# PRBonn/SHINE_mapping

Hardware: NVIDIA H100
Metric: sdf_train_points_per_sec_fwd_bwd (higher is better)
Workload: dtype f32

## Files before the change

### shine_mapping_b200/csrc/shine_b200.cu

```cuda

#include <cuda_runtime.h>
#include <math.h>
#include <stdint.h>

#include <type_traits>

#include "shine_b200.h"

#ifndef SHINE_GATHER_GROUP
#define SHINE_GATHER_GROUP 2
#endif
#ifndef SHINE_TRAIN_MINB
#define SHINE_TRAIN_MINB 2
#endif
#ifndef SHINE_TRAIN_DECGRAD_MINB
#define SHINE_TRAIN_DECGRAD_MINB 1
#endif
#ifndef SHINE_INFER_MINB
#define SHINE_INFER_MINB 3
#endif

#include "shine_device.cuh"

namespace {
// ... 205 lines not shown
                    acc.x = fmaf(w, v.x, acc.x); acc.y = fmaf(w, v.y, acc.y); acc.z = fmaf(w, v.z, acc.z); acc.w = fmaf(w, v.w, acc.w);
                } else {
                    red_add_f4(lv.feature_grads + (int64_t)ids[c] * F + 4 * part, w * d.x, w * d.y, w * d.z, w * d.w);
                }
            }
        }
    }
    if (MODE == 0) {
#pragma unroll
        for (int o = 1; o < LP; o <<= 1) {
            g3[0] += __shfl_xor_sync(kFull, g3[0], o); g3[1] += __shfl_xor_sync(kFull, g3[1], o); g3[2] += __shfl_xor_sync(kFull, g3[2], o);
        }
        if (valid && part == 0) { out[3 * p] = g3[0]; out[3 * p + 1] = g3[1]; out[3 * p + 2] = g3[2]; }
    } else if (MODE == 1) {
        if (valid) *reinterpret_cast<float4*>(out + p * F + 4 * part) = acc;
    }
}

__device__ __forceinline__ void to_afrag(const float (&v)[4], int odd, float (&a)[4]) {
    const float s0 = odd ? v[0] : v[2], s1 = odd ? v[1] : v[3];
    const float r0 = __shfl_xor_sync(kFull, s0, 1), r1 = __shfl_xor_sync(kFull, s1, 1);
    if (!odd) { a[0] = v[0]; a[2] = v[1]; a[1] = r0; a[3] = r1; }
    else      { a[0] = r0;   a[2] = r1;   a[1] = v[2]; a[3] = v[3]; }
}
__device__ __forceinline__ void from_cfrag(const float (&c)[4], int odd, float (&v)[4]) {
    const float s0 = odd ? c[0] : c[2], s1 = odd ? c[1] : c[3];
    const float r0 = __shfl_xor_sync(kFull, s0, 1), r1 = __shfl_xor_sync(kFull, s1, 1);
    if (!odd) { v[0] = c[0]; v[1] = c[1]; v[2] = r0; v[3] = r1; }
    else      { v[0] = r0;   v[1] = r1;   v[2] = c[2]; v[3] = c[3]; }
}

#define SHINE_ACC_DECL float dW2[2][4][4], dW1[2][4], db2p[4][2], db1p[4][2], dw3p[4][2]

__device__ __forceinline__ float reduce_scatter_g8(const float (&v)[8], int lane) {
    float a[4], b[2];
    const bool b4 = (lane & 16) != 0, b3 = (lane & 8) != 0, b2 = (lane & 4) != 0;
#pragma unroll
    for (int i = 0; i < 4; ++i) a[i] = (b4 ? v[4 + i] : v[i]) + __shfl_xor_sync(kFull, b4 ? v[i] : v[4 + i], 16);
#pragma unroll
    for (int i = 0; i < 2; ++i) b[i] = (b3 ? a[2 + i] : a[i]) + __shfl_xor_sync(kFull, b3 ? a[i] : a[2 + i], 8);
    return (b2 ? b[1] : b[0]) + __shfl_xor_sync(kFull, b2 ? b[0] : b[1], 4);
}

__device__ __forceinline__ int frag_chunk(int lane) { return lane ^ ((lane >> 2) & 6); }
template <int NTF>
__device__ __forceinline__ void load_afrag(const float* blk, int c, AFrag<NTF>& a) {
    const float4 v = *reinterpret_cast<const float4*>(blk + 4 * c);
    a.set_packed(v.x, v.y, v.z, v.w);
}
__device__ __forceinline__ void load_bfrag(const float* blk, int c, uint2& bh, uint2& bl) {
    const float2 v = *reinterpret_cast<const float2*>(blk + 2 * c);
    split_fast2(v.x, v.y, bh.x, bh.y, bl.x, bl.y);
}
__device__ __forceinline__ void stage_afrags(float* blk, const int (&sq)[2], const float (&c)[4][4]) {
#pragma unroll
    for (int mt = 0; mt < 2; ++mt)
#pragma unroll
        for (int q = 0; q < 2; ++q)
            *reinterpret_cast<float4*>(blk + 128 * mt + 4 * sq[q]) = make_float4(c[2 * mt][q], c[2 * mt + 1][q], c[2 * mt][2 + q], c[2 * mt + 1][2 + q]);
}
__device__ __forceinline__ int xfrag_word(int ks, int c) { return 64 * ks + 2 * (c ^ (8 * ks)); }
__device__ __forceinline__ void load_xfrag(const float* sx, int ks, int c, uint2& bh, uint2& bl) {
    const float2 v = *reinterpret_cast<const float2*>(sx + xfrag_word(ks, c));
    split_fast2(v.x, v.y, bh.x, bh.y, bl.x, bl.y);
}


constexpr int kGatherGroup = SHINE_GATHER_GROUP;

using shine_internal::StepParams;

struct SmemPlan {
    static constexpr int W1 = 0;
    static constexpr int W1T = W1 + 2 * kH * kF;
    static constexpr int W2 = W1T + 2 * kF * kWS;
    static constexpr int W3W2T = W2 + 2 * kH * kWS;
    static constexpr int B1 = W3W2T + 2 * kH * kWS;
    static constexpr int B2 = B1 + kH;
    static constexpr int W3 = B2 + kH;
    static constexpr int B3 = W3 + kH;
    static constexpr int GSCALE = B3 + 1;
    static constexpr int kDecGradFloats = kH * kF + kH + kH * kH + kH + kH + 1;
    static constexpr int ZSUM = B3 + 4;
    static constexpr int kZsumFloats = 8 * 5 * kTile;
    static constexpr int STAGE = ZSUM + kZsumFloats;
    static constexpr int SB2 = 0;
    static constexpr int SU = SB2;
    static constexpr int SA1 = SB2 + kTile * kH;
    static constexpr int SX = SA1 + kTile * kH;
    static constexpr int SA2 = SX + kTile * kF;
    static constexpr int SDP = SA2;
    static constexpr int kStagePerWarp = SA2 + kTile * kH;
    static constexpr int kStageGrouped = SDP + 2 * kTile;
    __host__ __device__ static constexpr int stage_per_warp(bool grouped) { return grouped ? kStageGrouped : kStagePerWarp; }
    static constexpr int kGroupPerLevel = 4 * kTile;
    static constexpr int kW2Part = kH * kH;
};

constexpr int kMaxGroupedRuns = 6;

__device__ __forceinline__ void red_add_f2(float* p, float a, float b) {
    asm volatile("red.global.add.v2.f32 [%0], {%1,%2};" ::"l"(p), "f"(a), "f"(b) : "memory");
}
__device__ __forceinline__ int group_slot(int p) { return 4 * (p & 3) + (p >> 2); }

template <int LMAX>
__device__ __forceinline__ void grouped_scatter(const StepParams& P, int L, int tile, const float* __restrict__ pt,
                                                float* __restrict__ dtile, const float (&dxc)[4], int lane) {
    const int g = lane >> 2, t = lane & 3;
    *reinterpret_cast<float2*>(dtile + g * kF + 2 * t) = make_float2(dxc[0], dxc[1]);
    *reinterpret_cast<float2*>(dtile + (g + 8) * kF + 2 * t) = make_float2(dxc[2], dxc[3]);
    __syncwarp();
    uint2 bh[2], bl[2];
#pragma unroll
    for (int c = 0; c < 2; ++c)
        split_fast2(dtile[(8 * c + t) * kF + g], dtile[(8 * c + t + 4) * kF + g], bh[c].x, bh[c].y, bl[c].x, bl[c].y);
    const float sx = (g & 4) ? 1.f : -1.f, ox = (g & 4) ? 0.f : 1.f;
    const float sy = (g & 2) ? 1.f : -1.f, oy = (g & 2) ? 0.f : 1.f;
    const float sz = (g & 1) ? 1.f : -1.f, oz = (g & 1) ? 0.f : 1.f;
    const int id_off = 8 * (g & 1) + 4 + (g >> 1);
    const int own = group_slot(lane & 15);
#pragma unroll
    for (int i = 0; i < LMAX; ++i) {
        if (i >= L) break;
        const float* lt = pt + i * SmemPlan::kGroupPerLevel;
        const int v_own = __float_as_int(lt[48 + own]);
        const uint32_t same = __match_any_sync(kFull, v_own);
        const int lead = __ffs(same) - 1;
        const uint32_t bmask = __ballot_sync(kFull, v_own >= 0 && lead == lane);
        if (bmask == 0) continue;
        const int rid_own = v_own >= 0 ? __popc(bmask & ((1u << lead) - 1u)) : 255;
        const shine_level& lv = P.oct.lv[i];
        const int32_t* slot_words = reinterpret_cast<const int32_t*>(lv.hash_slots);
        float* gb = grad_base(lv, (uint32_t)tile, kF);
        const int nruns = __popc(bmask);
        if (nruns > kMaxGroupedRuns) {
            const int odd = t & 1, half = t >> 1, mp = group_slot(g + 8 * odd);
            const int v = __float_as_int(lt[48 + mp]);
            if (v >= 0) {
                const float tx = lt[mp], ty = lt[16 + mp], tz = lt[32 + mp];
                const float ux = __fsub_rn(1.0f, tx), uy = __fsub_rn(1.0f, ty), uz = __fsub_rn(1.0f, tz);
                const int4 e = ldg_i4(slot_words + 16 * (int64_t)v + 4), o = ldg_i4(slot_words + 16 * (int64_t)v + 12);
                const int ids[8] = {e.x, o.x, e.y, o.y, e.z, o.z, e.w, o.w};
                const float4 d = *reinterpret_cast<const float4*>(dtile + (g + 8 * odd) * kF + 4 * half);
                const float xy[4] = {__fmul_rn(ux, uy), __fmul_rn(ux, ty), __fmul_rn(tx, uy), __fmul_rn(tx, ty)};
                const f2_t zz = f2_pack(uz, tz), d01 = f2_pack(d.x, d.y), d23 = f2_pack(d.z, d.w);
#pragma unroll
                for (int c = 0; c < 8; c += 2) {
                    float w[2];
                    f2_unpack(f2_mul(f2_pack(xy[c >> 1], xy[c >> 1]), zz), w[0], w[1]);
#pragma unroll
                    for (int k = 0; k < 2; ++k) {
                        const f2_t wk = f2_pack(w[k], w[k]);
                        float g0, g1, g2, g3;
                        f2_unpack(f2_mul(wk, d01), g0, g1); f2_unpack(f2_mul(wk, d23), g2, g3);
                        red_add_f4(gb + (int64_t)ids[c + k] * kF + 4 * half, g0, g1, g2, g3);
                    }
                }
            }
            continue;
        }
        const float4 tx4 = *reinterpret_cast<const float4*>(lt + 4 * t);
        const float4 ty4 = *reinterpret_cast<const float4*>(lt + 16 + 4 * t);
        const float4 tz4 = *reinterpret_cast<const float4*>(lt + 32 + 4 * t);
        float w[4];
        {
            const f2_t s_x = f2_pack(sx, sx), o_x = f2_pack(ox, ox), s_y = f2_pack(sy, sy), o_y = f2_pack(oy, oy);
            const f2_t s_z = f2_pack(sz, sz), o_z = f2_pack(oz, oz);
            const f2_t X01 = f2_fma(f2_pack(tx4.x, tx4.y), s_x, o_x), X23 = f2_fma(f2_pack(tx4.z, tx4.w), s_x, o_x);
            const f2_t Y01 = f2_fma(f2_pack(ty4.x, ty4.y), s_y, o_y), Y23 = f2_fma(f2_pack(ty4.z, ty4.w), s_y, o_y);
            const f2_t Z01 = f2_fma(f2_pack(tz4.x, tz4.y), s_z, o_z), Z23 = f2_fma(f2_pack(tz4.z, tz4.w), s_z, o_z);
            f2_unpack(f2_mul(f2_mul(X01, Y01), Z01), w[0], w[1]);
            f2_unpack(f2_mul(f2_mul(X23, Y23), Z23), w[2], w[3]);
        }
        int rid[4];
#pragma unroll
        for (int q = 0; q < 4; ++q) rid[q] = __shfl_sync(kFull, rid_own, t + 4 * q);
        uint32_t rem = bmask;
        for (int r = 0; r < nruns; r += 2) {
            const int p1 = __ffs(rem) - 1; rem &= rem - 1;
// ... 60 lines not shown
    const int g = lane >> 2, t = lane & 3, odd = t & 1, half = t >> 1;
    constexpr int kWarps = 8;

    for (int i = tid; i < kH * kF; i += blockDim.x) {
        const int nrow = i / kF, k = i % kF;
        uint32_t hi, lo; split_tf32(P.dec.w1[i], hi, lo);
        smu[SmemPlan::W1 + i] = hi; smu[SmemPlan::W1 + kH * kF + i] = lo;
        smu[SmemPlan::W1T + k * kWS + nrow] = hi; smu[SmemPlan::W1T + kF * kWS + k * kWS + nrow] = lo;
    }
    for (int i = tid; i < kH * kH; i += blockDim.x) {
        const int nrow = i / kH, k = i % kH;
        const float w = P.dec.w2[i];
        uint32_t hi, lo; split_tf32(w, hi, lo);
        smu[SmemPlan::W2 + nrow * kWS + k] = hi; smu[SmemPlan::W2 + kH * kWS + nrow * kWS + k] = lo;
        split_tf32(__fmul_rn(P.dec.w3[nrow], w), hi, lo);
        smu[SmemPlan::W3W2T + k * kWS + nrow] = hi; smu[SmemPlan::W3W2T + kH * kWS + k * kWS + nrow] = lo;
    }
    if (tid < kH) {
        smem[SmemPlan::B1 + tid] = P.dec.b1 ? P.dec.b1[tid] : 0.f;
        smem[SmemPlan::B2 + tid] = P.dec.b2 ? P.dec.b2[tid] : 0.f;
        smem[SmemPlan::W3 + tid] = P.dec.w3[tid];
    }
    if (tid == 0) {
        smem[SmemPlan::B3] = P.dec.b3 ? P.dec.b3[0] : 0.f;
        smem[SmemPlan::GSCALE] = P.loss_scale * ((TRAIN && P.d_loss) ? __ldg(P.d_loss) : 1.0f);
    }
    constexpr int kPark = LMAX <= 4 ? 16 : 32;
    constexpr int kIdPark = 4 * LMAX;
    __syncthreads();
    SHINE_ACC_DECL;
#pragma unroll
    for (int a = 0; a < 2; ++a) {
#pragma unroll
        for (int b = 0; b < 4; ++b) { dW2[a][b][0] = dW2[a][b][1] = dW2[a][b][2] = dW2[a][b][3] = 0.f; }
        dW1[a][0] = dW1[a][1] = dW1[a][2] = dW1[a][3] = 0.f;
    }
#pragma unroll
    for (int j = 0; j < 4; ++j) { db2p[j][0] = db2p[j][1] = db1p[j][0] = db1p[j][1] = dw3p[j][0] = dw3p[j][1] = 0.f; }
    float dw3acc = 0.f, db2acc[4] = {0.f, 0.f, 0.f, 0.f}, db1acc[2][2] = {{0.f, 0.f}, {0.f, 0.f}};

    constexpr bool kSectorProbe = !TRAIN;
    const bool poly = P.oct.poly_interp != 0;
    const int L = P.oct.num_levels;

    float db3p = 0.f;
    float loss_acc = 0.f;

    constexpr int kStage = SmemPlan::stage_per_warp(GROUPED);
    float* stage = smem + SmemPlan::STAGE + warp * kStage;
    float* stX = stage + SmemPlan::SX;
    const int kp = g >> 2, fc = frag_chunk(lane);
    const int sq[2] = {frag_chunk(8 * t + (g & 3)), frag_chunk(8 * t + 4 + (g & 3))};
    float* gpt = smem + SmemPlan::STAGE + (DEC_GRAD ? 8 * kStage : 0) +
                 warp * (LMAX * SmemPlan::kGroupPerLevel + (DEC_GRAD ? 0 : kTile * kF));
    float* gdx = DEC_GRAD ? stX : gpt + LMAX * SmemPlan::kGroupPerLevel;
    float* w2p = smem + SmemPlan::STAGE + 8 * kStage + 8 * LMAX * SmemPlan::kGroupPerLevel + warp * SmemPlan::kW2Part;
    if (DEC_GRAD && GROUPED) {
#pragma unroll
        for (int f = 0; f < 8; ++f) *reinterpret_cast<float4*>(w2p + 128 * f + 4 * lane) = make_float4(0.f, 0.f, 0.f, 0.f);
    }

    const int warp_global = blockIdx.x * kWarps + warp;
    const int warp_stride = gridDim.x * kWarps;

    bool consecutive = true;
#pragma unroll
    for (int i = 1; i < LMAX; ++i)
        if (i < L && P.oct.lv[i].level != P.oct.lv[0].level - i) consecutive = false;

    float nx = 0.f, ny = 0.f, nz = 0.f, nlab = 0.f, nwgt = 1.f;
    bool nvalid = false;
    auto prefetch_inputs = [&](int tl) {
        const int64_t p = (int64_t)tl * kTile + g + 8 * odd;
        nvalid = tl < P.num_tiles && p < P.n;
        if (nvalid) {
            src.load(P, p, nx, ny, nz);
            if (P.label) nlab = __ldg(P.label + p);
            if (P.weighted) nwgt = fabsf(__ldg(P.weight + p));
        }
    };
    prefetch_inputs(warp_global);

    int phase = 0;
    bool advance = false, last_pass = false;
    float pred0 = 0.f, zsum = 0.f;
    auto loss_point = [&](float pv, float lb, float wg, float& li, float& dp) {
        if constexpr (LOSS == kLossBce) {
            const float zt = __fdividef(1.0f, 1.0f + __expf(-__fdividef(lb, P.sigma)));
            const float e = __expf(-fabsf(pv));
            li = fmaxf(pv, 0.f) - pv * zt + __logf(1.0f + e);
            dp = 0.f;
            if (TRAIN) {
                const float rs = __fdividef(1.0f, 1.0f + e);
                const float sg = pv >= 0.f ? rs : e * rs;
                dp = (sg - zt) * wg * smem[SmemPlan::GSCALE];
            }
        } else {
            float dli;
            diff_point<LOSS>(pv, lb, P.scale, li, dli);
            dp = TRAIN ? dli * wg * smem[SmemPlan::GSCALE] : 0.f;
        }
    };
    for (int seq = warp_global;; seq = advance ? seq + warp_stride : seq) {
        if (last_pass) break;
        const int tile = seq;
        if (phase == 1 && seq >= P.num_tiles) {
            if constexpr (DEC_GRAD) {
#pragma unroll
                for (int o = 16; o > 0; o >>= 1) zsum += __shfl_xor_sync(kFull, zsum, o);
                if (lane == 0) smem[SmemPlan::ZSUM + warp] = zsum;
                __syncthreads();
                if (warp != 0) break;
                float tot = 0.f;
#pragma unroll
                for (int w = 0; w < kWarps; ++w) tot += smem[SmemPlan::ZSUM + w];
                if (tot == 0.f) break;
                zsum = tot;
                phase = 2;
            } else {
                break;
            }
        }
        const bool virt = phase != 1;
        last_pass = phase == 2;
        advance = !virt;
        const int64_t base = (int64_t)tile * kTile;
        const int64_t myp = base + g + 8 * odd;
        const bool valid = virt ? false : nvalid;
        const float x = nx, y = ny, z = nz, lab = nlab, wgt = nwgt;
        if (!virt) prefetch_inputs(seq + warp_stride);

        float feat[4];
        float pk[kPark];
        float idp[kIdPark];
        uint32_t hitmask = 0;
        if constexpr (kSectorProbe) {
        {
            float acc[8] = {0.f, 0.f, 0.f, 0.f, 0.f, 0.f, 0.f, 0.f};
#pragma unroll
            for (int i = 0; i < kPark; ++i) pk[i] = 0.f;
            const unsigned long long key0 = valid ? morton_of(x, y, z, P.oct.lv[0].level) : 0ull;
#pragma unroll
            for (int g0 = 0; g0 < LMAX; g0 += kGatherGroup) {
                SlotSector sec[kGatherGroup];
#pragma unroll
                for (int j = 0; j < kGatherGroup; ++j) {
                    const int i = g0 + j;
                    if (i < L && valid) {
                        const shine_level& lv = P.oct.lv[i];
                        const unsigned long long kq = consecutive ? (key0 >> (3 * i)) : morton_of(x, y, z, lv.level);
                        sec[j] = ldg_sector(reinterpret_cast<const HashSlot*>(lv.hash_slots),
                                            hash_key(kq) & (lv.hash_capacity - 1), half);
                    }
                }
#pragma unroll
                for (int j = 0; j < kGatherGroup; ++j) {
                    const int i = g0 + j;
                    bool hit = false;
                    if (i < L && valid) {
                        const shine_level& lv = P.oct.lv[i];
                        const unsigned long long kq = consecutive ? (key0 >> (3 * i)) : morton_of(x, y, z, lv.level);
                        hit = resolve_sector(reinterpret_cast<const HashSlot*>(lv.hash_slots), lv.hash_capacity - 1, kq, half,
                                             sec[j]);
                    }
                    idp[4 * i] = __int_as_float(hit ? sec[j].ids[0] : -1); idp[4 * i + 1] = __int_as_float(hit ? sec[j].ids[1] : -1);
                    idp[4 * i + 2] = __int_as_float(hit ? sec[j].ids[2] : -1); idp[4 * i + 3] = __int_as_float(hit ? sec[j].ids[3] : -1);
                    if (hit) {
                        const shine_level& lv = P.oct.lv[i];
                        hitmask |= 1u << i;
                        float r0[8], r1[8], r2[8], r3[8];
                        ldg_row8(lv.features + (int64_t)sec[j].ids[0] * kF, r0);
                        ldg_row8(lv.features + (int64_t)sec[j].ids[1] * kF, r1);
                        ldg_row8(lv.features + (int64_t)sec[j].ids[2] * kF, r2);
                        ldg_row8(lv.features + (int64_t)sec[j].ids[3] * kF, r3);
                        Blend b; b.init(x, y, z, lv.level, poly);
                        pk[3 * i] = b.tx; pk[3 * i + 1] = b.ty; pk[3 * i + 2] = b.tz;
                        const float wz = half ? b.tz : b.uz;
                        const float w0 = __fmul_rn(__fmul_rn(b.ux, b.uy), wz), w1 = __fmul_rn(__fmul_rn(b.ux, b.ty), wz);
                        const float w2 = __fmul_rn(__fmul_rn(b.tx, b.uy), wz), w3 = __fmul_rn(__fmul_rn(b.tx, b.ty), wz);
                        blend4(acc, r0, r1, r2, r3, w0, w1, w2, w3);
                    }
                }
            }
#pragma unroll
            for (int q = 0; q < 4; ++q) {
                const float send = half ? acc[q] : acc[4 + q];
                const float recv = __shfl_xor_sync(kFull, send, 2);
                feat[q] = (half ? acc[4 + q] : acc[q]) + recv;
            }
        }
        } else {
        int slot[LMAX];
        {
            constexpr int LH = LMAX / 2;
            const unsigned long long key0 = valid ? morton_of(x, y, z, P.oct.lv[0].level) : 0ull;
            unsigned long long kq[LH];
            uint4 kf[LH];
            int mine[LH];
#pragma unroll
            for (int j = 0; j < LH; ++j) {
                const int i = 2 * j + half;
                mine[j] = -1;
                if (i < L && valid) {
                    const shine_level& lv = P.oct.lv[i];
                    const HashSlot* slots = reinterpret_cast<const HashSlot*>(lv.hash_slots);
                    kq[j] = consecutive ? (key0 >> (3 * i)) : morton_of(x, y, z, lv.level);
                    mine[j] = (int)(hash_key(kq[j]) & (lv.hash_capacity - 1));
// ... 91 lines not shown
        if (DEC_GRAD) {
#pragma unroll
            for (int q = 0; q < 4; ++q) stX[xfrag_word(kp, frag_chunk(16 * half + 4 * q + (g & 3))) + odd] = feat[q];
        }
        float h1[4][4];
        uint32_t m1 = 0;
        {
            uint2 bh[4], bl[4];
#pragma unroll
            for (int j = 0; j < 4; ++j) {
                const float bA = smem[SmemPlan::B1 + 8 * j + 2 * t], bB = smem[SmemPlan::B1 + 8 * j + 2 * t + 1];
                h1[j][0] = bA; h1[j][1] = bB; h1[j][2] = bA; h1[j][3] = bB;
                const int off = (8 * j + g) * kF + 2 * t;
                bh[j] = *reinterpret_cast<const uint2*>(smu + SmemPlan::W1 + off);
                bl[j] = *reinterpret_cast<const uint2*>(smu + SmemPlan::W1 + kH * kF + off);
            }
            mma3x4<NTF>(h1, ax, bh, bl);
#pragma unroll
            for (int j = 0; j < 4; ++j) {
#pragma unroll
                for (int r = 0; r < 4; ++r) {
                    if (TRAIN && h1[j][r] > 0.f) m1 |= 1u << (4 * j + r);
                    h1[j][r] = fmaxf(h1[j][r], 0.f);
                }
                if (DEC_GRAD && !GROUPED) {
#pragma unroll
                    for (int q = 0; q < 2; ++q)
                        *reinterpret_cast<float2*>(stage + SmemPlan::SB2 + (4 * kp + j) * 64 + 2 * sq[q]) = make_float2(h1[j][q], h1[j][2 + q]);
                }
            }
            if (DEC_GRAD && GROUPED) stage_afrags(stage + SmemPlan::SU + 256 * kp, sq, h1);
        }
        float h2[4][4];
        {
#pragma unroll
            for (int j = 0; j < 4; ++j) {
                const float bA = smem[SmemPlan::B2 + 8 * j + 2 * t], bB = smem[SmemPlan::B2 + 8 * j + 2 * t + 1];
                h2[j][0] = bA; h2[j][1] = bB; h2[j][2] = bA; h2[j][3] = bB;
            }
#pragma unroll
            for (int kk = 0; kk < 4; ++kk) {
                AFrag<NTF> a; a.set(h1[kk][0], h1[kk][2], h1[kk][1], h1[kk][3]);
                uint2 bh[4], bl[4];
#pragma unroll
                for (int j = 0; j < 4; ++j) {
                    const int off = (8 * j + g) * kWS + 8 * kk + 2 * t;
                    bh[j] = *reinterpret_cast<const uint2*>(smu + SmemPlan::W2 + off);
                    bl[j] = *reinterpret_cast<const uint2*>(smu + SmemPlan::W2 + kH * kWS + off);
                }
                mma3x4<NTF>(h2, a, bh, bl);
            }
#pragma unroll
            for (int j = 0; j < 4; ++j) {
#pragma unroll
                for (int r = 0; r < 4; ++r) h2[j][r] = fmaxf(h2[j][r], 0.f);
            }
        }
        float w3a[4], w3b[4];
#pragma unroll
        for (int j = 0; j < 4; ++j) { w3a[j] = smem[SmemPlan::W3 + 8 * j + 2 * t]; w3b[j] = smem[SmemPlan::W3 + 8 * j + 2 * t + 1]; }
        float p0 = 0.f, p8 = 0.f;
#pragma unroll
        for (int j = 0; j < 4; ++j) {
            p0 = fmaf(h2[j][0], w3a[j], p0); p0 = fmaf(h2[j][1], w3b[j], p0);
            p8 = fmaf(h2[j][2], w3a[j], p8); p8 = fmaf(h2[j][3], w3b[j], p8);
        }
        p0 += __shfl_xor_sync(kFull, p0, 1); p0 += __shfl_xor_sync(kFull, p0, 2);
        p8 += __shfl_xor_sync(kFull, p8, 1); p8 += __shfl_xor_sync(kFull, p8, 2);
        const float b3 = smem[SmemPlan::B3];
        p0 += b3; p8 += b3;
        const float pown = odd ? p8 : p0;
        if (phase == 0) { pred0 = pown; phase = 1; continue; }
        if (P.pred && half == 0 && valid) P.pred[myp] = src.out(pown);

        if (P.label == nullptr) continue;

        float dpo = 0.f;
        if (valid) {
            float li;
            loss_point(pown, lab, wgt, li, dpo);
            if (half == 0) loss_acc += wgt * li;
        }
        if (!TRAIN) continue;
        if (phase == 2) dpo = (g == 0 && odd == 0) ? zsum : 0.f;

        const float dpx = __shfl_xor_sync(kFull, dpo, 1);
        const float dp0 = odd ? dpx : dpo, dp8 = odd ? dpo : dpx;
        float db1t[4][2], dw3t[4][2];
        if (DEC_GRAD) {
#pragma unroll
            for (int j = 0; j < 4; ++j) { dw3t[j][0] = dp0 * h2[j][0] + dp8 * h2[j][2];  dw3t[j][1] = dp0 * h2[j][1] + dp8 * h2[j][3]; }
        }
        if (DEC_GRAD && !GROUPED) {
            float dh2[4][4];
#pragma unroll
            for (int j = 0; j < 4; ++j) {
                dh2[j][0] = h2[j][0] > 0.f ? dp0 * w3a[j] : 0.f; dh2[j][1] = h2[j][1] > 0.f ? dp0 * w3b[j] : 0.f;
                dh2[j][2] = h2[j][2] > 0.f ? dp8 * w3a[j] : 0.f; dh2[j][3] = h2[j][3] > 0.f ? dp8 * w3b[j] : 0.f;
                db2p[j][0] += dh2[j][0] + dh2[j][2]; db2p[j][1] += dh2[j][1] + dh2[j][3];
            }
            stage_afrags(stage + SmemPlan::SA2 + 256 * kp, sq, dh2);
        }
        if (DEC_GRAD && GROUPED) {
            uint32_t mg = 0, mg8 = 0;
#pragma unroll
            for (int j = 0; j < 4; ++j)
#pragma unroll
                for (int q = 0; q < 2; ++q) {
                    mg |= (h2[j][q] > 0.f ? 1u : 0u) << (8 * j + 2 * t + q);
                    mg8 |= (h2[j][2 + q] > 0.f ? 1u : 0u) << (8 * j + 2 * t + q);
                }
            mg |= __shfl_xor_sync(kFull, mg, 1); mg8 |= __shfl_xor_sync(kFull, mg8, 1);
            mg |= __shfl_xor_sync(kFull, mg, 2); mg8 |= __shfl_xor_sync(kFull, mg8, 2);
            if (t == 0) {
                *reinterpret_cast<float2*>(stage + SmemPlan::SDP + 2 * g) = make_float2(dp0, __uint_as_float(mg));
                *reinterpret_cast<float2*>(stage + SmemPlan::SDP + 2 * (g + 8)) = make_float2(dp8, __uint_as_float(mg8));
            }
        }
        if (DEC_GRAD && t == 0) db3p += dp0 + dp8;

        float dh1[4][4];
        {
#pragma unroll
            for (int j = 0; j < 4; ++j) { dh1[j][0] = dh1[j][1] = dh1[j][2] = dh1[j][3] = 0.f; }
#pragma unroll
            for (int kk = 0; kk < 4; ++kk) {
                const uint32_t a[4] = {h2[kk][0] > 0.f ? kTf32One : 0u, h2[kk][2] > 0.f ? kTf32One : 0u,
                                       h2[kk][1] > 0.f ? kTf32One : 0u, h2[kk][3] > 0.f ? kTf32One : 0u};
                uint2 bh[4], bl[4];
#pragma unroll
                for (int j = 0; j < 4; ++j) {
                    const int off = (8 * j + g) * kWS + 8 * kk + 2 * t;
                    bh[j] = *reinterpret_cast<const uint2*>(smu + SmemPlan::W3W2T + off);
                    bl[j] = *reinterpret_cast<const uint2*>(smu + SmemPlan::W3W2T + kH * kWS + off);
                }
                mma2x4_exact_a<NTF>(dh1, a, bh, bl);
            }
#pragma unroll
            for (int j = 0; j < 4; ++j) {
                dh1[j][0] *= dp0; dh1[j][1] *= dp0; dh1[j][2] *= dp8; dh1[j][3] *= dp8;
#pragma unroll
                for (int r = 0; r < 4; ++r) dh1[j][r] = ((m1 >> (4 * j + r)) & 1u) ? dh1[j][r] : 0.f;
                if (DEC_GRAD) { db1t[j][0] = dh1[j][0] + dh1[j][2]; db1t[j][1] = dh1[j][1] + dh1[j][3]; }
            }
            if (DEC_GRAD) stage_afrags(stage + SmemPlan::SA1 + 256 * kp, sq, dh1);
        }
        float dxc[4] = {0.f, 0.f, 0.f, 0.f};
        {
            float dxo[4] = {0.f, 0.f, 0.f, 0.f};
#pragma unroll
            for (int kk = 0; kk < 4; kk += 2) {
                AFrag<NTF> a0, a1;
                a0.set(dh1[kk][0], dh1[kk][2], dh1[kk][1], dh1[kk][3]);
                a1.set(dh1[kk + 1][0], dh1[kk + 1][2], dh1[kk + 1][1], dh1[kk + 1][3]);
                const int off = g * kWS + 8 * kk + 2 * t;
                const uint2 bh0 = *reinterpret_cast<const uint2*>(smu + SmemPlan::W1T + off);
                const uint2 bl0 = *reinterpret_cast<const uint2*>(smu + SmemPlan::W1T + kF * kWS + off);
                const uint2 bh1 = *reinterpret_cast<const uint2*>(smu + SmemPlan::W1T + off + 8);
                const uint2 bl1 = *reinterpret_cast<const uint2*>(smu + SmemPlan::W1T + kF * kWS + off + 8);
                mma3x2<NTF>(dxc, dxo, a0, a1, bh0, bl0, bh1, bl1);
            }
#pragma unroll
            for (int r = 0; r < 4; ++r) dxc[r] += dxo[r];
        }

        if (DEC_GRAD && !GROUPED) {
#pragma unroll
// ... 51 lines not shown
                    const float4 v = *reinterpret_cast<const float4*>(w2p + 128 * (4 * mt + nt) + 4 * lane);
                    acc[nt][0] = v.x; acc[nt][1] = v.y; acc[nt][2] = v.z; acc[nt][3] = v.w;
                }
#pragma unroll
                for (int ks = 0; ks < 2; ++ks) {
                    uint2 b[4];
#pragma unroll
                    for (int nt = 0; nt < 4; ++nt) {
                        b[nt].x = (mk[ks][0] >> (8 * nt)) & 1u ? kTf32One : 0u;
                        b[nt].y = (mk[ks][1] >> (8 * nt)) & 1u ? kTf32One : 0u;
                    }
                    const float4 v = *reinterpret_cast<const float4*>(stage + SmemPlan::SU + (2 * ks + mt) * 128 + 4 * fc);
                    AFrag<NTF> af;
                    af.set_packed(v.x * dpk[ks][0], v.y * dpk[ks][0], v.z * dpk[ks][1], v.w * dpk[ks][1]);
                    mma2x4_exact_b<NTF>(acc, af, b);
                }
#pragma unroll
                for (int nt = 0; nt < 4; ++nt)
                    *reinterpret_cast<float4*>(w2p + 128 * (4 * mt + nt) + 4 * lane) = make_float4(acc[nt][0], acc[nt][1], acc[nt][2], acc[nt][3]);
            }
#pragma unroll
            for (int ks = 0; ks < 2; ++ks) {
                uint2 bh, bl;
                load_xfrag(stX, ks, fc, bh, bl);
                AFrag<NTF> a[2];
#pragma unroll
                for (int mt = 0; mt < 2; ++mt) {
                    const float4 av = *reinterpret_cast<const float4*>(stage + SmemPlan::SA1 + (2 * ks + mt) * 128 + 4 * fc);
                    db1acc[mt][0] += av.x + av.z; db1acc[mt][1] += av.y + av.w;
                    a[mt].set_packed(av.x, av.y, av.z, av.w);
                }
                mma3x2<NTF>(dW1[0], dW1[1], a[0], a[1], bh, bl, bh, bl);
            }
            __syncwarp();
        }

        if constexpr (GROUPED) {
            grouped_scatter<LMAX>(P, L, tile, gpt, gdx, dxc, lane);
            continue;
        }
        float dx[4];
        from_cfrag(dxc, odd, dx);
        const float (&qk)[kPark] = pk;
        const float (&qid)[kIdPark] = idp;
#pragma unroll
        for (int i = 0; i < LMAX; ++i) {
            int ids[8];
#pragma unroll
            for (int k = 0; k < 4; ++k) {
                const int mine = __float_as_int(qid[4 * i + k]);
                const int other = __shfl_xor_sync(kFull, mine, 2);
                ids[2 * k] = half ? other : mine;
                ids[2 * k + 1] = half ? mine : other;
            }
            if (i < L && ids[0] >= 0) {
                const shine_level& lv = P.oct.lv[i];
                Blend b;
                b.tx = qk[3 * i]; b.ty = qk[3 * i + 1]; b.tz = qk[3 * i + 2];
                b.ux = __fsub_rn(1.0f, b.tx); b.uy = __fsub_rn(1.0f, b.ty); b.uz = __fsub_rn(1.0f, b.tz);
                float* gb = grad_base(lv, (uint32_t)tile, kF) + 4 * half;
                const float xy[4] = {__fmul_rn(b.ux, b.uy), __fmul_rn(b.ux, b.ty), __fmul_rn(b.tx, b.uy), __fmul_rn(b.tx, b.ty)};
                const f2_t zz = f2_pack(b.uz, b.tz), dx01 = f2_pack(dx[0], dx[1]), dx23 = f2_pack(dx[2], dx[3]);
#pragma unroll
                for (int c = 0; c < 8; c += 2) {
                    float w[2];
                    f2_unpack(f2_mul(f2_pack(xy[c >> 1], xy[c >> 1]), zz), w[0], w[1]);
#pragma unroll
                    for (int k = 0; k < 2; ++k) {
                        const f2_t wk = f2_pack(w[k], w[k]);
                        float g0, g1, g2, g3;
                        f2_unpack(f2_mul(wk, dx01), g0, g1); f2_unpack(f2_mul(wk, dx23), g2, g3);
                        red_add_f4(gb + (int64_t)ids[c + k] * kF, g0, g1, g2, g3);
                    }
                }
            }
        }
    }

    if (P.loss && P.label) {
#pragma unroll
        for (int o = 16; o > 0; o >>= 1) loss_acc += __shfl_xor_sync(kFull, loss_acc, o);
        if (lane == 0 && loss_acc != 0.f) atomicAdd(P.loss, loss_acc * P.loss_scale);
    }
    if (DEC_GRAD && GROUPED) {
        float* part = stage;
        constexpr int oB1 = 256, oB2 = 288, oW3 = 320, oB3 = 352, kVec = 353;
#pragma unroll
        for (int mt = 0; mt < 2; ++mt) {
            *reinterpret_cast<float2*>(part + (16 * mt + g) * kF + 2 * t) = make_float2(dW1[mt][0], dW1[mt][1]);
            *reinterpret_cast<float2*>(part + (16 * mt + g + 8) * kF + 2 * t) = make_float2(dW1[mt][2], dW1[mt][3]);
#pragma unroll
            for (int r = 0; r < 2; ++r) {
                float d1 = db1acc[mt][r], d2 = db2acc[2 * mt + r];
#pragma unroll
                for (int o = 1; o < 4; o <<= 1) { d1 += __shfl_xor_sync(kFull, d1, o); d2 += __shfl_xor_sync(kFull, d2, o); }
                if (t == 0) { part[oB1 + 16 * mt + g + 8 * r] = d1; part[oB2 + 8 * (2 * mt + r) + g] = d2; }
            }
        }
        part[oW3 + 8 * (g >> 1) + 2 * t + (g & 1)] = dw3acc;
#pragma unroll
        for (int o = 16; o > 0; o >>= 1) db3p += __shfl_xor_sync(kFull, db3p, o);
        if (lane == 0) part[oB3] = db3p;
        __syncthreads();
        for (int i = tid; i < kVec + kH * kH; i += blockDim.x) {
            float v = 0.f;
            float* dst;
            if (i < kVec) {
#pragma unroll
                for (int w = 0; w < kWarps; ++w) v += smem[SmemPlan::STAGE + w * kStage + i];
                if (i < oB1) dst = P.dec.gw1 + i;
                else if (i < oB2) dst = P.dec.gb1 ? P.dec.gb1 + (i - oB1) : nullptr;
                else if (i < oW3) { v *= smem[SmemPlan::W3 + (i - oB2)]; dst = P.dec.gb2 ? P.dec.gb2 + (i - oB2) : nullptr; }
                else if (i < oB3) dst = P.dec.gw3 + (i - oW3);
                else dst = P.dec.gb3;
            } else {
                const int e = i - kVec, r = e / kH, c = e % kH;
                const int f = 128 * (4 * (c >> 4) + (r >> 3)) + 4 * (4 * (c & 7) + ((r & 7) >> 1)) + 2 * ((c >> 3) & 1) + (r & 1);
#pragma unroll
                for (int w = 0; w < kWarps; ++w) v += w2p[(w - warp) * SmemPlan::kW2Part + f];
                v *= smem[SmemPlan::W3 + r];
                dst = P.dec.gw2 + e;
            }
            if (v != 0.f && dst) atomicAdd(dst, v);
        }
    }
    if (DEC_GRAD && !GROUPED) {
        float* part = stage;
        constexpr int oW1 = 0, oB1 = 256, oW2 = 288, oB2 = 1312, oW3 = 1344, oB3 = 1376;
        __syncwarp();
#pragma unroll
        for (int mt = 0; mt < 2; ++mt) {
#pragma unroll
            for (int nt = 0; nt < 4; ++nt) {
                *reinterpret_cast<float2*>(part + oW2 + (16 * mt + g) * kH + 8 * nt + 2 * t) = make_float2(dW2[mt][nt][0], dW2[mt][nt][1]);
                *reinterpret_cast<float2*>(part + oW2 + (16 * mt + g + 8) * kH + 8 * nt + 2 * t) = make_float2(dW2[mt][nt][2], dW2[mt][nt][3]);
            }
            *reinterpret_cast<float2*>(part + oW1 + (16 * mt + g) * kF + 2 * t) = make_float2(dW1[mt][0], dW1[mt][1]);
            *reinterpret_cast<float2*>(part + oW1 + (16 * mt + g + 8) * kF + 2 * t) = make_float2(dW1[mt][2], dW1[mt][3]);
        }
#pragma unroll
        for (int j = 0; j < 4; ++j) {
#pragma unroll
            for (int q = 0; q < 2; ++q) {
                float a = db1p[j][q], b = db2p[j][q], c = dw3p[j][q];
#pragma unroll
                for (int o = 4; o < 32; o <<= 1) {
                    a += __shfl_xor_sync(kFull, a, o); b += __shfl_xor_sync(kFull, b, o); c += __shfl_xor_sync(kFull, c, o);
                }
                if (g == 0) {
                    part[oB1 + 8 * j + 2 * t + q] = a;
                    part[oB2 + 8 * j + 2 * t + q] = b;
                    part[oW3 + 8 * j + 2 * t + q] = c;
                }
            }
        }
#pragma unroll
        for (int o = 16; o > 0; o >>= 1) db3p += __shfl_xor_sync(kFull, db3p, o);
        if (lane == 0) part[oB3] = db3p;
        __syncthreads();
        for (int i = tid; i < SmemPlan::kDecGradFloats; i += blockDim.x) {
            float v = 0.f;
#pragma unroll
            for (int w = 0; w < kWarps; ++w) v += smem[SmemPlan::STAGE + w * kStage + i];
            if (v == 0.f) continue;
            float* dst;
            if (i < oB1) dst = P.dec.gw1 + i;
            else if (i < oW2) dst = P.dec.gb1 ? P.dec.gb1 + (i - oB1) : nullptr;
            else if (i < oB2) dst = P.dec.gw2 + (i - oW2);
            else if (i < oW3) dst = P.dec.gb2 ? P.dec.gb2 + (i - oB2) : nullptr;
            else if (i < oB3) dst = P.dec.gw3 + (i - oW3);
            else dst = P.dec.gb3;
            if (dst) atomicAdd(dst, v);
        }
    }
}


__global__ void __launch_bounds__(256) reduce_replicas_kernel(const __grid_constant__ shine_octree oct) {
    const shine_level& lv = oct.lv[blockIdx.y];
    if (lv.num_replicas <= 1 || !lv.grad_replicas || !lv.feature_grads) return;
    const int64_t n4 = (int64_t)lv.rows * oct.feature_dim / 4;
    float4* main4 = reinterpret_cast<float4*>(lv.feature_grads);
    float4* rep4 = reinterpret_cast<float4*>(lv.grad_replicas);
    const float4 zero = make_float4(0.f, 0.f, 0.f, 0.f);
    const int nrep = lv.num_replicas - 1;
    for (int64_t i = (int64_t)blockIdx.x * blockDim.x + threadIdx.x; i < n4; i += (int64_t)gridDim.x * blockDim.x) {
        float4 acc = main4[i];
        int r = 0;
        for (; r + 8 <= nrep; r += 8) {
            float4 v[8];
#pragma unroll
            for (int u = 0; u < 8; ++u) v[u] = rep4[(int64_t)(r + u) * n4 + i];
#pragma unroll
            for (int u = 0; u < 8; ++u) {
                acc.x += v[u].x; acc.y += v[u].y; acc.z += v[u].z; acc.w += v[u].w;
                rep4[(int64_t)(r + u) * n4 + i] = zero;
            }
        }
        for (; r < nrep; ++r) {
            const float4 v = rep4[(int64_t)r * n4 + i];
            acc.x += v.x; acc.y += v.y; acc.z += v.z; acc.w += v.w;
            rep4[(int64_t)r * n4 + i] = zero;
        }
        main4[i] = acc;
    }
}


struct AdamParams {
    shine_adam_tensor t[SHINE_ADAM_MAX_TENSORS];
    int32_t count;
    float beta1, beta2, omb1, omb2, eps, bc1, bc2_sqrt;
    int32_t zero_grad;
    const float* bc_dev;
};

struct AdamDevState { int32_t step; float bc1, bc2_sqrt; };

__global__ void adam_bump_kernel(AdamDevState* st, float beta1, float beta2) {
    const int step = st->step + 1;
    st->step = step;
    st->bc1 = (float)(1.0 - pow((double)beta1, (double)step));
    st->bc2_sqrt = (float)sqrt(1.0 - pow((double)beta2, (double)step));
}

__global__ void __launch_bounds__(256) adam_kernel(const __grid_constant__ AdamParams A) {
    const shine_adam_tensor& T = A.t[blockIdx.y];
    const int64_t n4 = T.numel >> 2;
    const float bc1 = A.bc_dev ? A.bc_dev[0] : A.bc1;
    const float bc2_sqrt = A.bc_dev ? A.bc_dev[1] : A.bc2_sqrt;
    const float step_size = T.lr / bc1;
    for (int64_t i = (int64_t)blockIdx.x * blockDim.x + threadIdx.x; i < n4; i += (int64_t)gridDim.x * blockDim.x) {
        float4 p = reinterpret_cast<float4*>(T.param)[i];
        float4 gr = reinterpret_cast<float4*>(T.grad)[i];
        float4 m = reinterpret_cast<float4*>(T.exp_avg)[i];
        float4 v = reinterpret_cast<float4*>(T.exp_avg_sq)[i];
        float* pp = &p.x; float* gg = &gr.x; float* mm = &m.x; float* vv = &v.x;
#pragma unroll
        for (int k = 0; k < 4; ++k) {
            float gk = gg[k];
            if (T.weight_decay != 0.f) gk = fmaf(T.weight_decay, pp[k], gk);
            mm[k] = mm[k] + (gk - mm[k]) * A.omb1;
            vv[k] = A.beta2 * vv[k] + A.omb2 * gk * gk;
            const float denom = sqrtf(vv[k]) / bc2_sqrt + A.eps;
            pp[k] -= step_size * (mm[k] / denom);
        }
// ... 375 lines not shown
```

Baseline: 4.156 billion.

## Fold zero-feature tile gradient into the final reduction analytically

Removes the extra virtual 'phase 2' tile pass that warp 0 ran after a block-wide sync to backpropagate the accumulated zero-input correction (zsum) through the decoder MLP. The zero-input gradient is now computed in closed form by one warp (a 32-wide hidden MLP evaluated at zero features), stored in spare shared memory, and added as zs*g0 during the final per-block atomic reduction. This drops a serialized tail pass and a mid-loop __syncthreads, at the cost of a small per-block matvec and extra shared-memory reads in the reduction. The numerics of the decoder gradient change slightly because of the different accumulation order.

New measurement: 4.314 billion, median of 6. 1.04x the previous value.

```diff
diff --git a/shine_mapping_b200/csrc/shine_b200.cu b/shine_mapping_b200/csrc/shine_b200.cu
--- a/shine_mapping_b200/csrc/shine_b200.cu
+++ b/shine_mapping_b200/csrc/shine_b200.cu
@@ -311,7 +311,12 @@
     static constexpr int GSCALE = B3 + 1;
     static constexpr int kDecGradFloats = kH * kF + kH + kH * kH + kH + kH + 1;
     static constexpr int ZSUM = B3 + 4;
+    static constexpr int H1Z = ZSUM + 8;
+    static constexpr int H2Z = H1Z + kH;
+    static constexpr int D2Z = H2Z + kH;
+    static constexpr int DB1Z = D2Z + kH;
     static constexpr int kZsumFloats = 8 * 5 * kTile;
+    static_assert(DB1Z + kH <= ZSUM + kZsumFloats, "g0 fits the zero-tile corner");
     static constexpr int STAGE = ZSUM + kZsumFloats;
     static constexpr int SB2 = 0;
     static constexpr int SU = SB2;
@@ -325,6 +330,31 @@
     static constexpr int kGroupPerLevel = 4 * kTile;
     static constexpr int kW2Part = kH * kH;
 };
+
+__device__ __forceinline__ void zero_tile_gradient(float* smem, const float* __restrict__ w2, int lane) {
+    const float h1 = fmaxf(smem[SmemPlan::B1 + lane], 0.f);
+    float a2 = smem[SmemPlan::B2 + lane];
+#pragma unroll
+    for (int k = 0; k < kH; ++k) a2 = fmaf(__ldg(w2 + lane * kH + k), __shfl_sync(kFull, h1, k), a2);
+    const float d2 = a2 > 0.f ? smem[SmemPlan::W3 + lane] : 0.f;
+    float db1 = 0.f;
+#pragma unroll
+    for (int n = 0; n < kH; ++n) db1 = fmaf(__ldg(w2 + n * kH + lane), __shfl_sync(kFull, d2, n), db1);
+    smem[SmemPlan::H1Z + lane] = h1;
+    smem[SmemPlan::H2Z + lane] = fmaxf(a2, 0.f);
+    smem[SmemPlan::D2Z + lane] = d2;
+    smem[SmemPlan::DB1Z + lane] = h1 > 0.f ? db1 : 0.f;
+}
+__device__ __forceinline__ float zero_tile_sum_and_gradient(float* smem, const float* __restrict__ w2, int warp, int lane) {
+    float s = 0.f;
+#pragma unroll
+    for (int w = 0; w < 8; ++w) s += smem[SmemPlan::ZSUM + w];
+    if (s != 0.f) {
+        if (warp == 0) zero_tile_gradient(smem, w2, lane);
+        __syncthreads();
+    }
+    return s;
+}
 
 constexpr int kMaxGroupedRuns = 6;
 
@@ -551,7 +581,8 @@
     prefetch_inputs(warp_global);
 
     int phase = 0;
-    bool advance = false, last_pass = false;
+    bool advance = false;
+    bool infer_exit = false;
     float pred0 = 0.f, zsum = 0.f;
     auto loss_point = [&](float pv, float lb, float wg, float& li, float& dp) {
         if constexpr (LOSS == kLossBce) {
@@ -571,27 +602,11 @@
         }
     };
     for (int seq = warp_global;; seq = advance ? seq + warp_stride : seq) {
-        if (last_pass) break;
+        if (!TRAIN && infer_exit) break;
         const int tile = seq;
-        if (phase == 1 && seq >= P.num_tiles) {
-            if constexpr (DEC_GRAD) {
-#pragma unroll
-                for (int o = 16; o > 0; o >>= 1) zsum += __shfl_xor_sync(kFull, zsum, o);
-                if (lane == 0) smem[SmemPlan::ZSUM + warp] = zsum;
-                __syncthreads();
-                if (warp != 0) break;
-                float tot = 0.f;
-#pragma unroll
-                for (int w = 0; w < kWarps; ++w) tot += smem[SmemPlan::ZSUM + w];
-                if (tot == 0.f) break;
-                zsum = tot;
-                phase = 2;
-            } else {
-                break;
-            }
-        }
+        if (phase == 1 && seq >= P.num_tiles) break;
         const bool virt = phase != 1;
-        last_pass = phase == 2;
+        if (!TRAIN) infer_exit = phase == 2;
         advance = !virt;
         const int64_t base = (int64_t)tile * kTile;
         const int64_t myp = base + g + 8 * odd;
@@ -849,7 +864,6 @@
             if (half == 0) loss_acc += wgt * li;
         }
         if (!TRAIN) continue;
-        if (phase == 2) dpo = (g == 0 && odd == 0) ? zsum : 0.f;
 
         const float dpx = __shfl_xor_sync(kFull, dpo, 1);
         const float dp0 = odd ? dpx : dpo, dp8 = odd ? dpo : dpx;
@@ -1067,6 +1081,11 @@
         for (int o = 16; o > 0; o >>= 1) loss_acc += __shfl_xor_sync(kFull, loss_acc, o);
         if (lane == 0 && loss_acc != 0.f) atomicAdd(P.loss, loss_acc * P.loss_scale);
     }
+    if (DEC_GRAD) {
+#pragma unroll
+        for (int o = 16; o > 0; o >>= 1) zsum += __shfl_xor_sync(kFull, zsum, o);
+        if (lane == 0) smem[SmemPlan::ZSUM + warp] = zsum;
+    }
     if (DEC_GRAD && GROUPED) {
         float* part = stage;
         constexpr int oB1 = 256, oB2 = 288, oW3 = 320, oB3 = 352, kVec = 353;
@@ -1087,25 +1106,30 @@
         for (int o = 16; o > 0; o >>= 1) db3p += __shfl_xor_sync(kFull, db3p, o);
         if (lane == 0) part[oB3] = db3p;
         __syncthreads();
+        const float zs = zero_tile_sum_and_gradient(smem, P.dec.w2, warp, lane);
         for (int i = tid; i < kVec + kH * kH; i += blockDim.x) {
-            float v = 0.f;
+            float v = 0.f, g0 = 0.f;
             float* dst;
             if (i < kVec) {
 #pragma unroll
                 for (int w = 0; w < kWarps; ++w) v += smem[SmemPlan::STAGE + w * kStage + i];
                 if (i < oB1) dst = P.dec.gw1 + i;
-                else if (i < oB2) dst = P.dec.gb1 ? P.dec.gb1 + (i - oB1) : nullptr;
-                else if (i < oW3) { v *= smem[SmemPlan::W3 + (i - oB2)]; dst = P.dec.gb2 ? P.dec.gb2 + (i - oB2) : nullptr; }
-                else if (i < oB3) dst = P.dec.gw3 + (i - oW3);
-                else dst = P.dec.gb3;
+                else if (i < oB2) { g0 = smem[SmemPlan::DB1Z + (i - oB1)]; dst = P.dec.gb1 ? P.dec.gb1 + (i - oB1) : nullptr; }
+                else if (i < oW3) {
+                    v *= smem[SmemPlan::W3 + (i - oB2)]; g0 = smem[SmemPlan::D2Z + (i - oB2)];
+                    dst = P.dec.gb2 ? P.dec.gb2 + (i - oB2) : nullptr;
+                } else if (i < oB3) { g0 = smem[SmemPlan::H2Z + (i - oW3)]; dst = P.dec.gw3 + (i - oW3); }
+                else { g0 = 1.f; dst = P.dec.gb3; }
             } else {
                 const int e = i - kVec, r = e / kH, c = e % kH;
                 const int f = 128 * (4 * (c >> 4) + (r >> 3)) + 4 * (4 * (c & 7) + ((r & 7) >> 1)) + 2 * ((c >> 3) & 1) + (r & 1);
 #pragma unroll
                 for (int w = 0; w < kWarps; ++w) v += w2p[(w - warp) * SmemPlan::kW2Part + f];
                 v *= smem[SmemPlan::W3 + r];
+                if (zs != 0.f) g0 = smem[SmemPlan::D2Z + r] * smem[SmemPlan::H1Z + c];
                 dst = P.dec.gw2 + e;
             }
+            if (zs != 0.f) v = fmaf(zs, g0, v);
             if (v != 0.f && dst) atomicAdd(dst, v);
         }
     }
@@ -1143,10 +1167,20 @@
         for (int o = 16; o > 0; o >>= 1) db3p += __shfl_xor_sync(kFull, db3p, o);
         if (lane == 0) part[oB3] = db3p;
         __syncthreads();
+        const float zs = zero_tile_sum_and_gradient(smem, P.dec.w2, warp, lane);
         for (int i = tid; i < SmemPlan::kDecGradFloats; i += blockDim.x) {
             float v = 0.f;
 #pragma unroll
             for (int w = 0; w < kWarps; ++w) v += smem[SmemPlan::STAGE + w * kStage + i];
+            if (zs != 0.f && i >= oB1) {
+                float g0;
+                if (i < oW2) g0 = smem[SmemPlan::DB1Z + (i - oB1)];
+                else if (i < oB2) g0 = smem[SmemPlan::D2Z + (i - oW2) / kH] * smem[SmemPlan::H1Z + (i - oW2) % kH];
+                else if (i < oW3) g0 = smem[SmemPlan::D2Z + (i - oB2)];
+                else if (i < oB3) g0 = smem[SmemPlan::H2Z + (i - oW3)];
+                else g0 = 1.f;
+                v = fmaf(zs, g0, v);
+            }
             if (v == 0.f) continue;
             float* dst;
             if (i < oB1) dst = P.dec.gw1 + i;
```
